# amolchanov86/gym_art

Measured on AMD Instinct MI355X. Metric: env-steps/sec (whole node) at N=2^20 Hummingbird; achieved HBM GB/s, higher is better.
Workload: dtype f64

## Files before the change

gym_art_amd/csrc/gaq.hip:

```cpp
#include "gaq_host.hpp"

#define GAQ_X(FEAT) extern template __global__ GAQ_STEP_SIG(FEAT)
GAQ_STEP_ALL(GAQ_X)
#undef GAQ_X
#define GAQ_X(FEAT) extern template __global__ GAQ_ROLL_SIG(FEAT)
GAQ_ROLL_ALL(GAQ_X)
#undef GAQ_X

namespace {

using namespace gaqk;

__global__ __launch_bounds__(kBlock) void episode_kernel(int64_t n, const float* __restrict__ reward,
                                                          const uint8_t* __restrict__ done, float* __restrict__ ep_ret,
                                                          uint32_t* __restrict__ ep_len, double* __restrict__ acc) {
  const int64_t i = (int64_t)blockIdx.x * kBlock + threadIdx.x;
  float ret = 0.0f; uint32_t len = 0; bool fin = false;
  if (i < n) {
    ret = ep_ret[i] + reward[i];
    len = ep_len[i] + 1u;
    fin = done[i] != 0;
    ep_ret[i] = fin ? 0.0f : ret;
    ep_len[i] = fin ? 0u : len;
  }
// ... 28 lines not shown
  for (int o = 32; o > 0; o >>= 1) acc += __shfl_down(acc, o);
  if ((threadIdx.x & 63) == 0) atomicAdd(reinterpret_cast<unsigned long long*>(out), (unsigned long long)acc);
}

__global__ __launch_bounds__(kBlock) void hbm_copy_kernel(const u32x4* __restrict__ src, u32x4* __restrict__ dst, size_t n16) {
  size_t i = (size_t)blockIdx.x * kBlock + threadIdx.x;
  const size_t stride = (size_t)gridDim.x * kBlock;
  for (; i < n16; i += stride) dst[i] = src[i];
}

__global__ void bump_kernel(uint64_t* ctr, uint64_t inc) { *ctr += inc; }
__global__ void fold_counter_kernel(uint64_t* ctr) {
  uint64_t sum = 0;
  for (int k = 0; k < kCtrSlots; ++k) { sum += ctr[k * kCtrStride]; ctr[k * kCtrStride] = 0; }
  ctr[0] = sum;
}

struct TileDirect {
  const DevPtrs& p; int64_t tile; uint32_t lane;
  __device__ __forceinline__ double ld64(const double* arr, int planes, int plane) const {
    auto r = __builtin_amdgcn_make_buffer_rsrc(const_cast<double*>(arr + tile * planes * kTile), 0, planes * kTile * 8, 0x00020000);
    return __builtin_bit_cast(double, __builtin_amdgcn_raw_buffer_load_b64(r, lane * 8u, plane * (kTile * 8), 0));
  }
  __device__ __forceinline__ void st64(double* arr, int planes, int plane, double v) const {
    auto r = __builtin_amdgcn_make_buffer_rsrc(arr + tile * planes * kTile, 0, planes * kTile * 8, 0x00020000);
    __builtin_amdgcn_raw_buffer_store_b64(__builtin_bit_cast(u32x2, v), r, lane * 8u, plane * (kTile * 8), 0);
  }
  __device__ __forceinline__ float ld32(const float* arr, int plane) const {
    auto r = __builtin_amdgcn_make_buffer_rsrc(const_cast<float*>(arr + tile * 4 * kTile), 0, kGrpBytes, 0x00020000);
    return __builtin_bit_cast(float, __builtin_amdgcn_raw_buffer_load_b32(r, lane * 4u, plane * (kTile * 4), 0));
// ... 27 lines not shown
      for (int k = 0; k < 18; ++k) v[k] = lo_decode(alias, p.obs_in, p.lo, i, k);
#pragma unroll
      for (int j = 0; j < 3; ++j) { s.pos[j] = v[j] + s.goal[j]; s.vel[j] = v[3 + j]; s.omega[j] = v[15 + j]; }
#pragma unroll
      for (int j = 0; j < 9; ++j) s.rot[j] = v[6 + j];
    } else {
#pragma unroll
      for (int j = 0; j < 3; ++j) { s.pos[j] = t.ld64(p.core, kCorePlanes, j); s.vel[j] = t.ld64(p.core, kCorePlanes, 3 + j);
                                    s.omega[j] = t.ld64(p.core, kCorePlanes, 15 + j); }
#pragma unroll
      for (int j = 0; j < 9; ++j) s.rot[j] = t.ld64(p.core, kCorePlanes, 6 + j);
    }
#pragma unroll
    for (int j = 0; j < 4; ++j) { s.rot_damp[j] = t.ld64(p.lag, kLagPlanes, j); s.cmds_damp[j] = t.ld32(p.cmds, j);
                                  s.ou[j] = t.ld32(p.ou, j); s.act_prev[j] = t.ld32(p.actp, j); }
    const uint32_t cw = p.ctr[i];
    s.tick = cw & 0xFFFFu; s.svd_ctr = cw >> 16;
    float acc[3] = {0.0f, 0.0f, 9.81f};
    float hist[4] = {s.act_prev[0], s.act_prev[1], s.act_prev[2], s.act_prev[3]};
    if (do_reset && (mask == nullptr || mask[i])) {
      gaq::reset_env<double, gaq::F_GENERIC>(s, cfg, cfg.env_offset + (uint64_t)i, cfg.step_index);
#pragma unroll
      for (int j = 0; j < 3; ++j) t.st32(p.goal, j, (float)s.goal[j]);
      if (!alias) {
#pragma unroll
        for (int j = 0; j < 3; ++j) { t.st64(p.core, kCorePlanes, j, s.pos[j]); t.st64(p.core, kCorePlanes, 3 + j, s.vel[j]);
                                      t.st64(p.core, kCorePlanes, 15 + j, s.omega[j]); }
#pragma unroll
        for (int j = 0; j < 9; ++j) t.st64(p.core, kCorePlanes, 6 + j, s.rot[j]);
      }
#pragma unroll
      for (int j = 0; j < 4; ++j) { t.st64(p.lag, kLagPlanes, j, s.rot_damp[j]); t.st32(p.cmds, j, s.cmds_damp[j]);
                                    t.st32(p.actp, j, s.act_prev[j]); }
      p.ctr[i] = (s.tick & 0xFFFFu) | (s.svd_ctr << 16);
      hist[0] = hist[1] = hist[2] = hist[3] = 0.0f;
    }
    float hi18[18];
#pragma unroll
    for (int k = 0; k < 18; ++k) hi18[k] = 0.0f;
    if (alias) {
      double v[18];
#pragma unroll
      for (int j = 0; j < 3; ++j) { v[j] = s.pos[j] - s.goal[j]; v[3 + j] = s.vel[j]; v[15 + j] = s.omega[j]; }
#pragma unroll
      for (int j = 0; j < 9; ++j) v[6 + j] = s.rot[j];
#pragma unroll
      for (int k = 0; k < 18; ++k) {
        if (alias == 2) { hi18[k] = (float)v[k]; }
        else { lo_encode(alias, p.lo, i, k, v[k]); hi18[k] = split_hi(v[k]); }
      }
// ... 364 lines not shown
    return fail(GAQ_ERR_STATE, "obs_state_alias: the observation tensor returned by the previous step / reset was modified before "
                               "this call -- it is the integrator state's fp32 head (include/gaq.h gaq_config.obs_state_alias); "
                               "copy it before editing, or create the handle with obs_state_alias = 2 (library-owned heads)");
  return GAQ_OK;
}

uint32_t launch_variant_of(const gaq_env* e) {
  const uint32_t v = (uint32_t)e->variant;
  if (e->d.rows_out && rows_twin_of(v) != 0xFFFFFFFFu) return rows_twin_of(v);
  if (e->d.step_ctr && ctr_twin_of(v) != 0xFFFFFFFFu) return ctr_twin_of(v);
  return v;
}

}

int launch_step(gaq_env* e, const float* actions, float* obs, float* reward, uint8_t* done, hipStream_t st) {
  e->info_valid = false;
  if ((reinterpret_cast<uintptr_t>(actions) & 15) != 0) return fail(GAQ_ERR_INVALID, "actions must be 16-byte aligned");
  if ((reinterpret_cast<uintptr_t>(obs) & 15) != 0) return fail(GAQ_ERR_INVALID, "obs must be 16-byte aligned");
  if (e->sc.noise == gaq::NOISE_INPUT) {
    if (!e->noise_next) return fail(GAQ_ERR_STATE, "GAQ_NOISE_INPUT: call gaq_set_noise_input_dev before each step");
    e->d.noise_in = e->noise_next;
    e->noise_next = nullptr;
  }
  if (e->sc.sense_input) {
    if (!e->sense_next) return fail(GAQ_ERR_STATE, "sense_input: call gaq_set_sense_input_dev before each step");
    e->d.sense_in = e->sense_next;
    e->sense_next = nullptr;
  }
  const int tiles_per_block = kBlock / kTile;
// ... 16 lines not shown
    const void* fn = step_kernel_ptr((uint32_t)e->variant);
    if (!fn || lds > 160 * 1024) return fail(GAQ_ERR_INVALID, "observation rows too large for the CU's LDS");
    HIP_TRY(hipFuncSetAttribute(fn, hipFuncAttributeMaxDynamicSharedMemorySize, (int)lds));
    e->lds_raised_for = e->variant;
  }
  const uint32_t launch_variant = launch_variant_of(e);
  if (e->d.rz_every > 0 && (launch_variant & gaq::F_RZ) != 0) {
    const bool hot_only = e->sc.compact_params != 0 && e->sc.zero_damp != 0 && (launch_variant & gaq::F_FP32) == 0;
    if (hot_only) e->cold_stale = true;
    else if (e->cold_stale) {
      if (int rc = launch_catch_up(e, st)) return rc;
    }
  }
  if (e->d.rz_every > 0 && e->rz_refill_now) { if (int rc = launch_refill(e, st)) return rc; }
  const bool self_counting = (launch_variant & gaq::F_CTR) != 0;
  if (e->d.step_ctr && !self_counting) {
    bool capturing = false;
    hipStreamCaptureStatus cs = hipStreamCaptureStatusNone;
    if (hipStreamIsCapturing(st, &cs) == hipSuccess) capturing = cs == hipStreamCaptureStatusActive; else (void)hipGetLastError();
    if (e->ctr_spread || capturing) {
      hipLaunchKernelGGL(fold_counter_kernel, dim3(1), dim3(1), 0, st, e->d.step_ctr);
      HIP_TRY(hipGetLastError());
      if (!capturing) e->ctr_spread = false;
    }
  }
  if (launch_variant != e->noted_step) { launch_record().note(0, launch_variant); e->noted_step = launch_variant; }
#define GAQ_LAUNCH(FEAT) \
  hipLaunchKernelGGL(step_kernel<(FEAT)>, grid, block, lds, st, e->d, e->sc, e->um, actions, obs, reward, done, lpw)
  switch (launch_variant) {
#define GAQ_X(FEAT) case (int)(FEAT): GAQ_LAUNCH(FEAT); break;
    GAQ_STEP_ALL(GAQ_X)
#undef GAQ_X
    default: return fail(GAQ_ERR_STATE, "internal: no kernel instantiation for this feature mask");
  }
// ... 116 lines not shown
float* mirror_aux(const gaq_env* e, char* base) { return reinterpret_cast<float*>(base + planes_bytes(e)); }

char* device_view(char* pinned) {
  void* dp = nullptr;
  if (hipHostGetDevicePointer(&dp, pinned, 0) == hipSuccess && dp) return static_cast<char*>(dp);
  (void)hipGetLastError();
  return nullptr;
}

int export_state(gaq_env* e, double* planes_dst, float* aux_dst, hipStream_t st) {
  if (!planes_dst) {
    if (!e->export_dev) HIP_TRY(hipMalloc((void**)&e->export_dev, planes_bytes(e)));
    planes_dst = e->export_dev;
  }
  if (e->alias) e->d.obs_in = e->last_obs;
  const dim3 grid((unsigned)((e->d.n + kBlock - 1) / kBlock)), block(kBlock);
  hipLaunchKernelGGL(export_kernel, grid, block, 0, st, e->d, alias_mode(e), planes_dst, aux_dst);
  HIP_TRY(hipGetLastError());
  return GAQ_OK;
}

int mirror_info(gaq_env* e) {
  if (!e->info_pin) {
    const bool mapped = e->stage_map != nullptr;
    HIP_TRY(hipHostMalloc((void**)&e->info_pin, planes_bytes(e) + aux_bytes(e), mapped ? hipHostMallocMapped : hipHostMallocDefault));
    if (mapped) e->info_map = device_view(e->info_pin);
  }
  if (e->info_map) return export_state(e, mirror_planes(e->info_map), mirror_aux(e, e->info_map), e->stream);
  if (int rc = export_state(e, nullptr, nullptr, e->stream)) return rc;
  HIP_TRY(hipMemcpyAsync(mirror_planes(e->info_pin), e->export_dev, planes_bytes(e), hipMemcpyDeviceToHost, e->stream));
// ... 81 lines not shown
    derive_model(cfg->model, dt, e->um);
    e->um.jinv = nullptr;
    if (cfg->control == GAQ_CTRL_MELLINGER && !inverse_jacobian(cfg->model, sc.jinv)) {
      delete e;
      return fail(GAQ_ERR_INVALID, "singular quadrotor jacobian");
    }
  } else {
    std::memset(&e->um, 0, sizeof(e->um));
  }
  { const ParamFlags f = start_flags(*cfg, e->um); e->any_lag = f.lag; e->any_drag = f.drag; }
  { const char* nf = getenv("GAQ_NO_FUSED"); if (nf && nf[0] == '1') e->fused_rollout = false; }
  e->ov = read_overrides();
  e->lomix = cfg->per_env_params != 0 || e->any_lag;
  { const char* ca = getenv("GAQ_CHECK_ALIAS"); e->check_alias = ca && ca[0] == '1'; }
  { const int sw = env_override("GAQ_SWEEP"); sc.sweep = sw < 0 ? kSweepDefault : sw; }
  {
    const char* ab = getenv("GAQ_ABLATE");
    sc.ablate = ab ? atoi(ab) : 0;
    if (sc.ablate != 0 && !kDiagBuild) {
      delete e;
      return fail(GAQ_ERR_INVALID, "GAQ_ABLATE is set but this libgaq is not a measurement build (make EXTRA=-DGAQ_DIAG_BUILD OUT=...): "
                                   "the ablations skip parts of the step and give wrong physics; unset the variable");
    }
    if (sc.ablate != 0) fprintf(stderr, "libgaq: GAQ_ABLATE=%d in a measurement build -- results are WRONG by construction, only timings mean anything\n", sc.ablate);
  }
  refresh_feature_flags(e);
  if (e->fp32 && !e->alias) {
    delete e;
    return fail(GAQ_ERR_INVALID, "fp32_state needs the specialised kernels (18-word world-frame obs, RawControl, default reward terms)");
  }
// ... 20 lines not shown
  if (e->alias) {
    if (!e->fp32) alloc0((void**)&d.lo, nt * (e->lomix ? (size_t)kMixRowsBytes : (size_t)kLoRowsBytes));
    alloc0((void**)&e->own_obs, nt * kRowsBytes);
  } else {
    alloc0((void**)&d.core, nt * kCoreBytes);
  }
  alloc0((void**)&d.lag, nt * kLagBytes);
  alloc0((void**)&d.ou, nt * kGrpBytes);
  alloc0((void**)&d.cmds, nt * kGrpBytes);
  alloc0((void**)&d.actp, nt * kGrpBytes);
  alloc0((void**)&d.goal, nt * kGrpBytes);
  alloc0((void**)&d.gyro, nt * kGrpBytes);
  alloc0((void**)&e->step_ctr_mem, sizeof(uint64_t) * kCtrSlots * kCtrStride);
  alloc0((void**)&e->alias_sum_dev, sizeof(uint64_t));
  alloc0((void**)&d.ctr, nt * kTile * sizeof(uint32_t));
  alloc0((void**)&d.done_count, sizeof(uint32_t) * 2);
  alloc0((void**)&d.nan_count, sizeof(uint32_t));
  if (cfg->compact_done) alloc0((void**)&d.done_list, nt * kTile * sizeof(uint32_t));
  if (cfg->aux_outputs) alloc0((void**)&d.aux, nt * kTile * gaq::AUX_WORDS * sizeof(float));
  if (cfg->per_env_params) {
    double* par = nullptr;
    double* jinv_dev = nullptr;
    alloc0((void**)&par, nt * kParBytes);
    if (cfg->control == GAQ_CTRL_MELLINGER) alloc0((void**)&jinv_dev, nt * kTile * 16 * sizeof(double));
    d.par = par;
    d.jinv = jinv_dev;
    alloc0((void**)&d.traj, 4 * nt * kTile * sizeof(uint32_t));
    d.rcount = d.traj ? d.traj + nt * kTile : nullptr;
    d.rz_flag = d.traj ? d.traj + 2 * nt * kTile : nullptr;
    e->host_par.assign(nt * kPar * kTile, 1.0);
// ... 40 lines not shown
    if (cfg->per_env_params)
      HIP_TRY(hipMemcpy(const_cast<double*>(d.par), e->host_par.data(), e->host_par.size() * sizeof(double), hipMemcpyHostToDevice));
    return GAQ_OK;
  };
  if (int rc = init_state()) { gaq_destroy(e); return rc; }
  *out = e;
  return GAQ_OK;
}

int gaq_destroy(gaq_env* e) {
  if (!e) return GAQ_OK;
  (void)hipSetDevice(e->cfg.device);
  if (e->stream) (void)hipStreamSynchronize(e->stream);
  (void)hipDeviceSynchronize();
  (void)hipFree(e->d.core); (void)hipFree(e->d.lo); (void)hipFree(e->own_obs); (void)hipFree(e->d.lag); (void)hipFree(e->d.ou); (void)hipFree(e->d.cmds);
  (void)hipFree(e->d.actp); (void)hipFree(e->d.goal); (void)hipFree(e->d.gyro); (void)hipFree(e->step_ctr_mem); if (e->info_pin) (void)hipHostFree(e->info_pin); (void)hipFree(e->alias_sum_dev); (void)hipFree(e->d.ctr);
  (void)hipFree(e->d.done_count); (void)hipFree(e->d.nan_count); (void)hipFree(e->d.done_list);
  (void)hipFree(e->d.ep_ret); (void)hipFree(e->d.ep_len); (void)hipFree(e->d.ep_acc); (void)hipFree(e->d.aux);
  (void)hipFree(const_cast<double*>(e->d.par)); (void)hipFree(const_cast<double*>(e->d.jinv));
  (void)hipFree(e->d.traj); (void)hipFree(e->d.rz_overrun);
  (void)hipFree(e->stage_dev); (void)hipFree(e->export_dev);
  if (e->stage_pin) (void)hipHostFree(e->stage_pin);
  if (e->ev0) (void)hipEventDestroy(e->ev0);
  if (e->ev1) (void)hipEventDestroy(e->ev1);
  if (e->stream) (void)hipStreamDestroy(e->stream);
  delete e;
  return GAQ_OK;
}

int gaq_is_diag_build(void) { return kDiagBuild ? 1 : 0; }

// ... 267 lines not shown
        lo_encode(mode, lo.data(), i, k, v);
      }
    HIP_TRY(hipMemcpy(e->own_obs, hi.data(), hi.size() * 4, hipMemcpyHostToDevice));
    if (!e->fp32) HIP_TRY(hipMemcpy(e->d.lo, lo.data(), lo.size(), hipMemcpyHostToDevice));
    e->last_obs = e->own_obs;
  } else {
    HIP_TRY(hipMemcpy(e->d.core, core.data(), core.size() * 8, hipMemcpyHostToDevice));
  }
  HIP_TRY(hipMemcpy(e->d.lag, lag.data(), lag.size() * 8, hipMemcpyHostToDevice));
  HIP_TRY(hipMemcpy(e->d.ou, ou.data(), ou.size() * 4, hipMemcpyHostToDevice));
  HIP_TRY(hipMemcpy(e->d.cmds, cmds.data(), cmds.size() * 4, hipMemcpyHostToDevice));
  HIP_TRY(hipMemcpy(e->d.actp, actp.data(), actp.size() * 4, hipMemcpyHostToDevice));
  HIP_TRY(hipMemcpy(e->d.goal, goal.data(), goal.size() * 4, hipMemcpyHostToDevice));
  HIP_TRY(hipMemcpy(e->d.gyro, gyro.data(), gyro.size() * 4, hipMemcpyHostToDevice));
  HIP_TRY(hipMemcpy(e->d.ctr, c.data(), c.size() * 4, hipMemcpyHostToDevice));
  e->rz_refill_now = true;
  return GAQ_OK;
}

int gaq_done_list(gaq_env* e, uint32_t* idx_out, int64_t capacity, int64_t* count_out) {
  if (!e || !count_out) return fail(GAQ_ERR_INVALID, "null argument");
  if (!e->d.done_list) return fail(GAQ_ERR_STATE, "handle was created with compact_done = 0");
  HIP_TRY(hipSetDevice(e->cfg.device));
  HIP_TRY(hipStreamSynchronize(e->stream));
  if (int rc_ = sync_handle(e)) return rc_;
  uint64_t step = e->sc.step_index;
  if (e->d.step_ctr) { if (int rc_ = read_step_counter(e, &step)) return rc_; }
  if (step == 0) { *count_out = 0; return GAQ_OK; }
  uint32_t cnt = 0;
  HIP_TRY(hipMemcpy(&cnt, e->d.done_count + ((step - 1) & 1), sizeof(uint32_t), hipMemcpyDeviceToHost));
// ... 167 lines not shown
```

gym_art_amd/csrc/gaq_host.hpp:

```cpp
#pragma once

#include <hip/hip_runtime.h>

#include <algorithm>
#include <cmath>
#include <cstdio>
#include <cstdlib>
#include <cstring>
#include <functional>
#include <mutex>
#include <new>
#include <set>
#include <string>
#include <vector>

#include "gaq_kernels.hpp"
#include "../../include/gaq.h"

using namespace gaqk;

namespace {
struct Randomizer {
  int32_t sampler, every;
  double ratio[gaq::TL_COUNT];
// ... 24 lines not shown
  int lds_raised_for = -1; bool reset_lds_raised = false;
  hipStream_t user_stream = nullptr;
  bool user_stream_used = false;
  const float* sense_next = nullptr;
  std::vector<double> host_par;
  bool dev_params = false;
  bool rz_on = false;
  bool cold_stale = false;
  int rz_since_refill = 0;
  bool rz_refill_now = false;
  Randomizer rz;
  std::vector<uint8_t> pflags;
  int64_t cnt_lag = 0, cnt_drag = 0, cnt_noncompact = 0, cnt_damp = 0;
  bool any_lag = false, any_drag = false;
  Overrides ov;
  bool ctr_spread = false;
  int num_cus = 256;
  int variant = 0;
  int lds_per_wave = 0;
  bool needs_generic = false;
  bool fused_rollout = true;
  bool alias = false;
  bool pack = false;
  bool shadow = false;
  bool check_alias = false;
  uint64_t* alias_sum_dev = nullptr;
  uint64_t alias_sum = 0; bool alias_sum_valid = false;
  bool lomix = false;
  bool fp32 = false;
  float* own_obs = nullptr;
// ... 15 lines not shown
      return fail(GAQ_ERR_DEVICE, std::string(#expr) + ": " + hipGetErrorString(e_));      \
  } while (0)

struct LaunchRecord {
  std::mutex mu;
  std::set<uint32_t> seen[3];
  void note(int kind, uint32_t f) { std::lock_guard<std::mutex> g(mu); seen[kind].insert(f); }
};
LaunchRecord& launch_record();

int fail(int code, const std::string& msg);
int env_override(const char* name);
int launch_step(gaq_env* e, const float* actions, float* obs, float* reward, uint8_t* done, hipStream_t st);
uint32_t fused_variant(const gaq_env* e);
int fused_rollout(gaq_env* e, int32_t T, float* obs, hipStream_t st, const std::function<int()>& launch);
int sync_handle(gaq_env* e);
int check_overrun(gaq_env* e);
void refresh_feature_flags(gaq_env* e);

void derive_model(const gaq_model& g, double dt, Model<double>& m);
bool inverse_jacobian(const gaq_model& g, double out[16]);
int check_model(const gaq_model& g);
int launch_refill(gaq_env* e, hipStream_t st);
int launch_jinv(gaq_env* e, hipStream_t st, const uint8_t* done);
int launch_catch_up(gaq_env* e, hipStream_t st);
int rebuild_params(gaq_env* e);

struct Scratch {
  void* p = nullptr;
  ~Scratch() { if (p) (void)hipFree(p); }
// ... 12 lines not shown
```

gym_art_amd/csrc/gaq_kernels.hpp:

```cpp
#pragma once

#include <hip/hip_runtime.h>

#include <cstddef>
#include <cstdint>

#include "../../include/gaq.h"
#include "quad_core.hpp"
#include "quad_params_dev.hpp"

namespace gaqk {

#ifndef GAQ_LD_AUX
#define GAQ_LD_AUX 0
#endif
#ifndef GAQ_ST_AUX
#define GAQ_ST_AUX 0
#endif
#ifndef GAQ_ACT_AUX
#define GAQ_ACT_AUX 0
#endif
#ifndef GAQ_ACTION_AUX
#define GAQ_ACTION_AUX GAQ_ACT_AUX
#endif
// ... 27 lines not shown
constexpr int kLoRowsLds = 3 * 1024;
constexpr int kMixRowWords = 11;
constexpr int kMixRowBytes = kMixRowWords * 4;
constexpr int kMixRowsBytes = kTile * kMixRowBytes;
template <uint32_t F> constexpr bool kLoMix = (F & (gaq::F_PER_ENV | gaq::F_LAG)) != 0;
constexpr int kPar = 45;
constexpr int kParBytes = kPar * kTile * 8;
constexpr int kHotPlanes = 19;
constexpr int kParNextSkew = 544;
enum ParPlane { PP_MASS = 0, PP_INV_MASS = 1, PP_INERTIA = 2, PP_INV_INERTIA = 5, PP_THRUST_MAX = 8, PP_TORQUE_MAX = 12,
                PP_PROP_X = 16, PP_PROP_Y = 20, PP_PROP_Z = 24, PP_TAU_UP = 28, PP_TAU_DOWN = 29, PP_LINEARITY = 30,
                PP_ARM = 31, PP_VEL_DAMP = 32, PP_DAMP_Q = 33, PP_C_DRAG = 34, PP_C_ROLL = 35, PP_OU_SIGMA = 36,
                PP_T2T = 37, PP_MX = 38, PP_MY = 39, PP_COMX = 40, PP_COMY = 41, PP_COMPACT_OK = 42,
                PP_T_UP = 43, PP_T_DOWN = 44 };

struct DevPtrs {
  double* core;
  void* lo;
  const float* obs_in;
  float* obs_copy;
  float* hi_final;
  double* lag;
  float* ou;
  float* cmds;
  float* actp;
  float* goal;
  float* gyro;
  uint32_t* ctr;
  const double* par;
  const double* jinv;
  const float* noise_in;
  const float* sense_in;
  float* aux;
  uint32_t* done_list;
  uint32_t* done_count;
  uint32_t* nan_count;
  float* term_obs;
  float* ep_ret;
  uint32_t* ep_len;
  double* ep_acc;
  uint64_t* step_ctr;
  uint32_t ctr_shift;
  uint32_t ctr_inc0;
// ... 9 lines not shown

using gaq::EnvState;
using gaq::Model;
using gaq::StepCfg;

template <uint32_t F> struct RealOf { using type = double; };
#define GAQ_REAL_FP32(FEAT) template <> struct RealOf<(FEAT)> { using type = float; };
GAQ_REAL_FP32(48u) GAQ_REAL_FP32(49u) GAQ_REAL_FP32(50u) GAQ_REAL_FP32(51u) GAQ_REAL_FP32(52u) GAQ_REAL_FP32(53u) GAQ_REAL_FP32(54u) GAQ_REAL_FP32(55u)
#undef GAQ_REAL_FP32
template <uint32_t F> using Real = typename RealOf<F>::type;

typedef unsigned int u32x2 __attribute__((ext_vector_type(2)));
typedef unsigned int u32x4 __attribute__((ext_vector_type(4)));
typedef __attribute__((address_space(3))) void lds_void;

struct TileImage { int lo, lag, ou, cmds, actp, goal, gyro, total; };

template <uint32_t F>
__host__ __device__ __forceinline__ TileImage tile_image(const StepCfg& cfg) {
  TileImage t;
  t.lo = kRowsLds;
  int o = (F & gaq::F_FP32) ? kRowsLds : (F & gaq::F_ALIAS) ? kRowsLds + kLoRowsLds : kCoreBytes;
  t.lag = o;  if (gaq::has_lag<F>(cfg)) o += kLagBytes;
  t.ou = o;   if (gaq::noise_mode<F>(cfg) != gaq::NOISE_OFF) o += kGrpBytes;
  t.cmds = o; if (gaq::has_lag<F>(cfg)) o += kGrpBytes;
  t.actp = o; if (gaq::has_act_prev<F>(cfg)) o += kGrpBytes;
  t.goal = o; if (gaq::has_env_goal<F>(cfg)) o += kGrpBytes;
  t.gyro = o; if (gaq::has_gyro_bias<F>(cfg)) o += kGrpBytes;
  t.total = o;
  return t;
// ... 506 lines not shown
template <uint32_t F> constexpr int kArgPrologue = 2;
#define GAQ_ARG_PROLOGUE(FEAT, FORM) template <> inline constexpr int kArgPrologue<(FEAT)> = (FORM);
GAQ_ARG_PROLOGUE(66578u, 1) GAQ_ARG_PROLOGUE(66577u, 1) GAQ_ARG_PROLOGUE(68627u, 1) GAQ_ARG_PROLOGUE(19477u, 1) GAQ_ARG_PROLOGUE(197653u, 1)
GAQ_ARG_PROLOGUE(197654u, 1) GAQ_ARG_PROLOGUE(197655u, 1) GAQ_ARG_PROLOGUE(199699u, 1)
#undef GAQ_ARG_PROLOGUE
template <uint32_t F, int FORM = 2, typename C, typename A>
__device__ __forceinline__ C kernarg_batch(uint32_t token, C carry, const DevPtrs& p, A actions, int lds_per_wave) {
  if constexpr (FORM == 1) {
    asm("s_waitcnt lgkmcnt(0)" : "+s"(carry) : "s"(token), "s"(p.ntiles), "s"(p.n), "s"(p.step_ctr));
    return carry;
  }
  if constexpr ((F & gaq::F_GENERIC) == 0) {
    if constexpr ((F & gaq::F_LAG) != 0) asm("" : "+s"(carry) : "s"(p.lag), "s"(p.cmds));
    if constexpr ((F & gaq::F_NOISE) != 0) asm("" : "+s"(carry) : "s"(p.ou));
  }
  if constexpr ((F & gaq::F_ALIAS) != 0) {
    asm("s_waitcnt lgkmcnt(0)" : "+s"(carry) : "s"(token), "s"(p.ntiles), "s"(p.n), "s"(p.step_ctr), "s"(p.ctr_shift), "s"(p.obs_in), "s"(p.lo),
        "s"(p.ctr), "s"(actions), "s"(lds_per_wave));
  } else {
    asm("s_waitcnt lgkmcnt(0)" : "+s"(carry) : "s"(token), "s"(p.ntiles), "s"(p.n), "s"(p.step_ctr), "s"(p.ctr_shift), "s"(p.core), "s"(p.ctr),
        "s"(actions), "s"(lds_per_wave));
  }
  return carry;
}

template <uint32_t F> constexpr int kStepMinWaves = 1;
#ifndef GAQ_NO_FLOORS
template <> inline constexpr int kStepMinWaves<214036u> = 3;
template <> inline constexpr int kStepMinWaves<82962u> = 3;
#endif
constexpr uint32_t kXcds = 8;
template <uint32_t F> constexpr bool kSweeps = true;
template <> inline constexpr bool kSweeps<17428u> = false;
template <> inline constexpr bool kSweeps<2569u> = false;
template <uint32_t F>
__global__ __launch_bounds__(kBlock) __attribute__((amdgpu_waves_per_eu(kStepMinWaves<F>))) void step_kernel(DevPtrs p, StepCfg cfg, Model<double> um,
// ... 15 lines not shown
      const uint32_t nblocks = (uint32_t)((p.ntiles + (kBlock / kTile - 1)) / (kBlock / kTile));
      const uint32_t xcd = block % kXcds, members = (nblocks - xcd + (kXcds - 1u)) / kXcds;
      const uint32_t mirrored = xcd + (members - 1u - block / kXcds) * kXcds;
      block = ((uint32_t)cfg.sweep & (uint32_t)cfg.step_index & 1u) != 0 ? mirrored : block;
    }
  }
  const int64_t tile = (int64_t)block * (kBlock / kTile) + wave;
  if constexpr ((F & gaq::F_CTR) != 0) {
    if (tile >= p.ntiles) {
      (void)step_counter_checkin(p, step_counter_read(p, lane), lane);
      return;
    }
  } else {
    if (tile >= p.ntiles) return;
  }
  char* buf = smem + wave * lds_per_wave;
  const int64_t i = tile * kTile + lane;
  const bool live = i < p.n;
  const int D = cfg.obs_dim;

  stage_in<F>(p, cfg, tile, buf, lane);
  if constexpr (kArgPrologue<F> == 2) __builtin_amdgcn_sched_barrier(0);
  using T = Real<F>;
  Model<T> m;
  if constexpr (!gaq::kModelMem<F>) load_model<F>(p, cfg, tile, lane, um, m);
  const Model<T>* mp = &m;
  if constexpr (gaq::kModelMem<F>) mp = (const Model<T>*)kernarg_model_ptr();
  float4 a4;
  uint32_t cw;
  {
    auto ra = __builtin_amdgcn_make_buffer_rsrc(const_cast<float*>(actions), 0, (int)(p.n * 16), 0x00020000);
    const u32x4 v = __builtin_amdgcn_raw_buffer_load_b128(ra, (uint32_t)i * 16u, 0, (F & gaq::F_NT) ? 2 : GAQ_ACTION_AUX);
    a4 = __builtin_bit_cast(float4, v);
    auto rc = __builtin_amdgcn_make_buffer_rsrc(p.ctr, 0, (int)(p.ntiles * kTile * 4), 0x00020000);
    cw = __builtin_amdgcn_raw_buffer_load_b32(rc, (uint32_t)i * 4u, 0, (F & gaq::F_NT) ? 2 : GAQ_ACT_AUX);
  }
  if constexpr ((F & gaq::F_CTR) != 0) cfg.step_index = step_counter_checkin(p, step_counter_read(p, lane), lane);
  float pre0[4] = {0.0f, 0.0f, 0.0f, 0.0f}, pre1[4] = {0.0f, 0.0f, 0.0f, 0.0f};
  if constexpr ((F & gaq::F_PREDRAW) != 0) {
    const gaq::Philox r0(cfg.seed, cfg.env_offset + (uint64_t)i, cfg.step_index, gaq::RNG_OU0);
    gaq::normals4(r0, pre0);
    if (cfg.sim_steps > 1) { const gaq::Philox r1(cfg.seed, cfg.env_offset + (uint64_t)i, cfg.step_index, gaq::RNG_OU0 + 1u); gaq::normals4(r1, pre1); }
  }
  if constexpr ((F & gaq::F_PREDRAW) != 0) {
    asm volatile("" :: "v"(pre0[0]), "v"(pre0[1]), "v"(pre0[2]), "v"(pre0[3]), "v"(pre1[0]), "v"(pre1[1]), "v"(pre1[2]), "v"(pre1[3]));
  }
  wait_dma();
  EnvState<T> s;
  read_image<F>(cfg, buf, lane, s);
  s.tick = cw & 0xFFFFu;
// ... 66 lines not shown
#pragma unroll
        for (int j = 0; j < 4; ++j) s.ou[j] = 0.0f;
      }
    }
  }
  if constexpr (kObsRowsInLds) {
    wave_lds_fence();
    if constexpr (A) flush_obs(p.obs_copy, p.n, D, tile, rows, lane);
    else flush_obs(obs, p.n, D, tile, rows, lane);
    if constexpr (kAuxRowsInLds) { if (p.aux) flush_obs(p.aux, p.n, gaq::AUX_WORDS, tile, rows + aux_off, lane); }
    wave_lds_fence();
  }
  write_image<F>(cfg, buf, lane, s);
  wave_lds_fence();
  stage_out<F>(p, cfg, tile, buf, lane, obs);
  {
    auto rc = __builtin_amdgcn_make_buffer_rsrc(p.ctr, 0, (int)(p.ntiles * kTile * 4), 0x00020000);
    __builtin_amdgcn_raw_buffer_store_b32((s.tick & 0xFFFFu) | (s.svd_ctr << 16), rc, (uint32_t)i * 4u, 0, kStAux<F>);
  }
  if (live) {
    if constexpr (GAQ_OUT_NT != 0) { __builtin_nontemporal_store(out.reward, &reward[i]); __builtin_nontemporal_store(out.done, &done[i]); }
    else { reward[i] = out.reward; done[i] = out.done; }
    if (!isfinite(out.reward)) atomicAdd(p.nan_count, 1u);
  }
  if constexpr (!gaq::kHeadsAreObs<F> && !kObsRowsInLds) {
    float* obs_rows_out = obs;
    if constexpr (A) obs_rows_out = p.obs_copy;
    wave_lds_fence();
    float* row = reinterpret_cast<float*>(rows) + lane * D;
    if (D == 18) {
#pragma unroll
// ... 169 lines not shown
  if (p.step_ctr) cfg.step_index = step_counter_peek(p, lane);
  const int64_t tile = (int64_t)blockIdx.x * (kBlock / kTile) + wave;
  if (tile >= p.ntiles) return;
  char* buf = smem + wave * lds_per_wave;
  const int64_t i = tile * kTile + lane;
  const bool live = i < p.n;
  const int64_t first = tile * kTile;
  const uint32_t nlive = (uint32_t)((p.n - first) < kTile ? (p.n - first) : kTile);
  const TileImage im = tile_image<F>(cfg);

  stage_in<F>(p, cfg, tile, buf, lane);
  __builtin_amdgcn_sched_barrier(0);
  using RT = Real<F>;
  Model<RT> m;
  load_model<F, true>(p, cfg, tile, lane, um, m);
  auto rc = __builtin_amdgcn_make_buffer_rsrc(p.ctr, 0, (int)(p.ntiles * kTile * 4), 0x00020000);
  const uint32_t cw = __builtin_amdgcn_raw_buffer_load_b32(rc, (uint32_t)i * 4u, 0, 0);
  auto load_action = [&](int t) {
    auto ra = __builtin_amdgcn_make_buffer_rsrc(const_cast<float*>(actions + ((int64_t)t * p.n + first) * 4), 0,
                                                (int)(nlive * 16u), 0x00020000);
    return __builtin_amdgcn_raw_buffer_load_b128(ra, lane * 16u, 0, 0);
  };
  u32x4 a_next = load_action(0);
  wait_dma();
  EnvState<RT> s;
  read_image<F>(cfg, buf, lane, s);
  s.tick = cw & 0xFFFFu;
  s.svd_ctr = cw >> 16;
  wave_lds_fence();
  StepCfg c = cfg;
  for (int t = 0; t < T; ++t) {
    const float4 a4 = __builtin_bit_cast(float4, a_next);
// ... 38 lines not shown
    wave_lds_fence();
    c.step_index += 1;
  }
  write_image<F>(cfg, buf, lane, s);
  wave_lds_fence();
  if (p.hi_final) copy_out_rows<5, kRowsBytes>(p.hi_final + first * 18, buf, lane, nlive * kRowBytes);
  if constexpr ((F & gaq::F_FP32) == 0) {
    if constexpr (kLoMix<F>) copy_out_rows<3, kMixRowsBytes>(reinterpret_cast<uint32_t*>(p.lo) + first * kMixRowWords, buf + im.lo, lane, kMixRowsBytes);
    else copy_out_rows<3, kLoRowsBytes>(reinterpret_cast<int16_t*>(p.lo) + first * 18, buf + im.lo, lane, kLoRowsBytes);
  }
  if (gaq::has_lag<F>(cfg)) {
    copy_out<2>(p.lag + tile * (kLagPlanes * kTile), buf + im.lag, lane);
    copy_out<1>(p.cmds + tile * (4 * kTile), buf + im.cmds, lane);
  }
  if (gaq::noise_mode<F>(cfg) != gaq::NOISE_OFF) copy_out<1>(p.ou + tile * (4 * kTile), buf + im.ou, lane);
  __builtin_amdgcn_raw_buffer_store_b32((s.tick & 0xFFFFu) | (s.svd_ctr << 16), rc, (uint32_t)i * 4u, 0, 0);
}

template <uint32_t F>
__device__ __forceinline__ void policy_rollout_body(const DevPtrs& p, StepCfg cfg, const Model<double>& um, int T, float* obs,
                                                    float* __restrict__ reward, uint8_t* __restrict__ done, char* buf, int64_t tile,
                                                    uint32_t lane, const PolicyDev* pol, float* pol_scratch, float* __restrict__ act_out) {
  const int64_t i = tile * kTile + lane;
  const bool live = i < p.n;
  const int64_t first = tile * kTile;
  const uint32_t nlive = (uint32_t)((p.n - first) < kTile ? (p.n - first) : kTile);
  const TileImage im = tile_image<F>(cfg);

  stage_in<F>(p, cfg, tile, buf, lane);
  using RT = Real<F>;
  Model<RT> m;
  load_model<F, true>(p, cfg, tile, lane, um, m);
  auto rc = __builtin_amdgcn_make_buffer_rsrc(p.ctr, 0, (int)(p.ntiles * kTile * 4), 0x00020000);
  const uint32_t cw = __builtin_amdgcn_raw_buffer_load_b32(rc, (uint32_t)i * 4u, 0, 0);
  wait_dma();
  EnvState<RT> s;
  read_image<F>(cfg, buf, lane, s);
  s.tick = cw & 0xFFFFu;
  s.svd_ctr = cw >> 16;
  wave_lds_fence();
  StepCfg c = cfg;
  for (int t = 0; t < T; ++t) {
    float act[4];
    policy_eval(*pol, reinterpret_cast<const float*>(buf + lane * kRowBytes), pol_scratch, lane, c.seed, c.env_offset + (uint64_t)i,
                c.step_index, act);
    if (act_out && live) {
      const u32x4 v = __builtin_bit_cast(u32x4, make_float4(act[0], act[1], act[2], act[3]));
      auto ro = __builtin_amdgcn_make_buffer_rsrc(act_out + ((int64_t)t * p.n + first) * 4, 0, (int)(nlive * 16u), 0x00020000);
      __builtin_amdgcn_raw_buffer_store_b128(v, ro, lane * 16u, 0, 0);
// ... 37 lines not shown
    wave_lds_fence();
    c.step_index += 1;
  }
  write_image<F>(cfg, buf, lane, s);
  wave_lds_fence();
  if (p.hi_final) copy_out_rows<5, kRowsBytes>(p.hi_final + first * 18, buf, lane, nlive * kRowBytes);
  if constexpr ((F & gaq::F_FP32) == 0) {
    if constexpr (kLoMix<F>) copy_out_rows<3, kMixRowsBytes>(reinterpret_cast<uint32_t*>(p.lo) + first * kMixRowWords, buf + im.lo, lane, kMixRowsBytes);
    else copy_out_rows<3, kLoRowsBytes>(reinterpret_cast<int16_t*>(p.lo) + first * 18, buf + im.lo, lane, kLoRowsBytes);
  }
  if (gaq::has_lag<F>(cfg)) {
    copy_out<2>(p.lag + tile * (kLagPlanes * kTile), buf + im.lag, lane);
    copy_out<1>(p.cmds + tile * (4 * kTile), buf + im.cmds, lane);
  }
  if (gaq::noise_mode<F>(cfg) != gaq::NOISE_OFF) copy_out<1>(p.ou + tile * (4 * kTile), buf + im.ou, lane);
  __builtin_amdgcn_raw_buffer_store_b32((s.tick & 0xFFFFu) | (s.svd_ctr << 16), rc, (uint32_t)i * 4u, 0, 0);
}

constexpr int kPolBlock = kTile;
template <uint32_t F>
__global__ __launch_bounds__(kPolBlock) void policy_rollout_kernel(DevPtrs p, StepCfg cfg, Model<double> um, int T, PolicyDev pol,
                                                                   float* __restrict__ act_out, float* obs, float* __restrict__ reward,
                                                                   uint8_t* __restrict__ done, int lds_per_wave) {
  static_assert((F & gaq::F_ALIAS) != 0 && (F & gaq::F_GENERIC) == 0, "fused rollout: alias layout only");
  extern __shared__ __attribute__((aligned(16))) char smem[];
  const uint32_t lane = threadIdx.x & 63u;
  const int64_t tile = kernarg_batch<F>(kernarg_warm(), (int64_t)blockIdx.x, p, act_out, lds_per_wave);
  if (p.step_ctr) cfg.step_index = step_counter_peek(p, lane);
  if (tile >= p.ntiles) return;
  float* scratch = reinterpret_cast<float*>(smem + ((lds_per_wave + 15) & ~15));
  policy_rollout_body<F>(p, cfg, um, T, obs, reward, done, smem, tile, lane, &pol, scratch, act_out);
// ... 41 lines not shown
```

gym_art_amd/csrc/gaq_params.hip:

```cpp
#include "gaq_host.hpp"

namespace {

dim3 grid_for(int64_t count) { return dim3((unsigned)((count + kBlock - 1) / kBlock)); }

__global__ __launch_bounds__(kBlock) void clear_dynamics_kernel(DevPtrs p, const int64_t* __restrict__ idx, int64_t first, int64_t count) {
  const int64_t k = (int64_t)blockIdx.x * kBlock + threadIdx.x;
  if (k >= count) return;
  const int64_t i = idx ? idx[k] : first + k;
  p.ctr[i] &= 0xFFFFu;
  float* ou = p.ou + (i / kTile) * (4 * kTile) + (i % kTile);
#pragma unroll
  for (int j = 0; j < 4; ++j) ou[j * kTile] = 0.0f;
}

__device__ __forceinline__ uint32_t* pfull_of(const DevPtrs& p) { return p.traj + 3 * p.ntiles * kTile; }

struct PlaneDest { double* base; int lane, stride; };
__device__ __forceinline__ PlaneDest env_planes(const DevPtrs& p, int64_t i) {
  return {const_cast<double*>(p.par) + (i / kTile) * (int64_t)(kPar * kTile), (int)(i % kTile), kTile};
}
__device__ __forceinline__ PlaneDest plane_row(double* row) { return {row, 0, 1}; }

__device__ __forceinline__ void write_model_planes(const PlaneDest& to, double dt, const gaq::DerivedModel& dm) {
// ... 342 lines not shown
    std::sort(tiles.begin(), tiles.end());
    tiles.erase(std::unique(tiles.begin(), tiles.end()), tiles.end());
    for (size_t a = 0; a < tiles.size();) {
      size_t b = a + 1;
      while (b < tiles.size() && tiles[b] == tiles[b - 1] + 1) ++b;
      HIP_TRY(hipMemcpy(const_cast<double*>(e->d.par) + (size_t)tiles[a] * kPar * kTile, hp + (size_t)tiles[a] * kPar * kTile,
                        (b - a) * (size_t)kParBytes, hipMemcpyHostToDevice));
      a = b;
    }
  }
  Scratch di;
  if (idx) {
    if (di.alloc(sizeof(int64_t) * (size_t)count)) return GAQ_ERR_DEVICE;
    HIP_TRY(hipMemcpy(di.p, idx, sizeof(int64_t) * (size_t)count, hipMemcpyHostToDevice));
  }
  hipLaunchKernelGGL(clear_dynamics_kernel, grid_for(count), dim3(kBlock), 0, e->stream, e->d, (const int64_t*)di.p, first, count);
  HIP_TRY(hipGetLastError());
  HIP_TRY(hipStreamSynchronize(e->stream));
  flags_from_counts(e);
  return GAQ_OK;
}

int need_device_params(gaq_env* e) {
  if (!e) return fail(GAQ_ERR_INVALID, "null handle");
  if (!e->cfg.per_env_params) return fail(GAQ_ERR_STATE, "handle was created with per_env_params = 0");
  return GAQ_OK;
}
int check_tree(const gaq_quad_params& t, bool by_density = false) {
  const double* v = reinterpret_cast<const double*>(&t);
  for (int k = 0; k < GAQ_TREE_DOUBLES; ++k) if (!std::isfinite(v[k])) return fail(GAQ_ERR_INVALID, "parameter tree: non-finite leaf");
// ... 55 lines not shown
  }
  e->d.rz_every = e->d.par_next ? rz->every : 0;
  e->rz_refill_now = true;
  const uint8_t nf = rz->sampler == 2 ? (uint8_t)PF_LAG : tree_flags(rz->base, e->sc.dt);
  for (int64_t i = 0; i < e->d.n; ++i) set_env_flags(e, i, nf);
  flags_from_counts(e);
  return GAQ_OK;
}

int gaq_randomize_dev(gaq_env* e, const uint8_t* mask_dev, void* stream) {
  if (int rc = need_device_params(e)) return rc;
  e->info_valid = false;
  if (!e->rz_on) return fail(GAQ_ERR_STATE, "no randomizer installed (gaq_set_randomizer)");
  HIP_TRY(hipSetDevice(e->cfg.device));
  e->user_stream = (hipStream_t)stream; e->user_stream_used = true;
  hipLaunchKernelGGL(params_redraw_kernel, grid_for(e->d.n), dim3(kBlock), 0, (hipStream_t)stream, e->d, e->sc, e->rz, mask_dev);
  HIP_TRY(hipGetLastError());
  if (int rc = launch_jinv(e, (hipStream_t)stream, nullptr)) return rc;
  if (e->d.rz_every > 0) return launch_refill(e, (hipStream_t)stream);
  return GAQ_OK;
}

int gaq_set_param_trees(gaq_env* e, const gaq_quad_params* trees, int32_t links_by_density, int64_t first, int64_t count) {
  if (int rc = need_device_params(e)) return rc;
  e->info_valid = false;
  if (!trees) return fail(GAQ_ERR_INVALID, "null argument");
  if (int rc = check_range(e, first, count)) return rc;
  if (count == 0) return GAQ_OK;
  if (!e->dev_params && (e->cnt_lag | e->cnt_drag | e->cnt_noncompact | e->cnt_damp) != 0)
    return fail(GAQ_ERR_STATE, "this handle already holds host-supplied parameters (gaq_set_params): do not mix the two paths");
  for (int64_t k = 0; k < count; ++k) if (int rc = check_tree(trees[k], links_by_density != 0)) return rc;
  HIP_TRY(hipSetDevice(e->cfg.device));
  if (int rc_ = sync_handle(e)) return rc_;
  Scratch dt_;
  if (dt_.alloc(sizeof(gaq_quad_params) * (size_t)count)) return GAQ_ERR_DEVICE;
  HIP_TRY(hipMemcpy(dt_.p, trees, sizeof(gaq_quad_params) * (size_t)count, hipMemcpyHostToDevice));
  hipLaunchKernelGGL(derive_trees_kernel, grid_for(count), dim3(kBlock), 0, e->stream, e->d, e->sc, (const double*)dt_.p, (int)links_by_density, first, count);
  HIP_TRY(hipGetLastError());
  e->dev_params = true;
  if (int rc = launch_jinv(e, e->stream, nullptr)) return rc;
  HIP_TRY(hipStreamSynchronize(e->stream));
  for (int64_t k = 0; k < count; ++k) set_env_flags(e, first + k, tree_flags(trees[k], e->sc.dt));
  flags_from_counts(e);
  return GAQ_OK;
}

int gaq_get_params(gaq_env* e, gaq_model* out, int64_t first, int64_t count) {
  if (!e || !out) return fail(GAQ_ERR_INVALID, "null argument");
  if (!e->cfg.per_env_params) return fail(GAQ_ERR_STATE, "handle was created with per_env_params = 0");
  if (int rc = check_range(e, first, count)) return rc;
  if (count == 0) return GAQ_OK;
// ... 46 lines not shown
```

Before: 22.62 billion.

## Elide per-env counter traffic with per-tile uniform counter headers

```diff
diff --git a/gym_art_amd/csrc/gaq.hip b/gym_art_amd/csrc/gaq.hip
--- a/gym_art_amd/csrc/gaq.hip
+++ b/gym_art_amd/csrc/gaq.hip
@@ -66,6 +66,16 @@
   uint64_t sum = 0;
   for (int k = 0; k < kCtrSlots; ++k) { sum += ctr[k * kCtrStride]; ctr[k * kCtrStride] = 0; }
   ctr[0] = sum;
+}
+
+__global__ __launch_bounds__(kBlock) void ctr_materialise_kernel(DevPtrs p) {
+  const int64_t i = (int64_t)blockIdx.x * kBlock + threadIdx.x;
+  const int64_t tile = i / kTile;
+  if (tile >= p.ntiles) return;
+  const CtrHdr h = p.ctr_hdr[tile];
+  if (h.uniform == 0) return;
+  p.ctr[i] = h.cw;
+  if (i % kTile == 0) const_cast<CtrHdr*>(p.ctr_hdr)[tile] = CtrHdr{0u, 0u};
 }
 
 struct TileDirect {
@@ -123,7 +133,8 @@
 #pragma unroll
     for (int j = 0; j < 4; ++j) { s.rot_damp[j] = t.ld64(p.lag, kLagPlanes, j); s.cmds_damp[j] = t.ld32(p.cmds, j);
                                   s.ou[j] = t.ld32(p.ou, j); s.act_prev[j] = t.ld32(p.actp, j); }
-    const uint32_t cw = p.ctr[i];
+    const CtrHdr ch = p.ctr_hdr[tile];
+    const uint32_t cw = ch.uniform ? ch.cw : p.ctr[i];
     s.tick = cw & 0xFFFFu; s.svd_ctr = cw >> 16;
     float acc[3] = {0.0f, 0.0f, 9.81f};
     float hist[4] = {s.act_prev[0], s.act_prev[1], s.act_prev[2], s.act_prev[3]};
@@ -141,8 +152,11 @@
 #pragma unroll
       for (int j = 0; j < 4; ++j) { t.st64(p.lag, kLagPlanes, j, s.rot_damp[j]); t.st32(p.cmds, j, s.cmds_damp[j]);
                                     t.st32(p.actp, j, s.act_prev[j]); }
-      p.ctr[i] = (s.tick & 0xFFFFu) | (s.svd_ctr << 16);
       hist[0] = hist[1] = hist[2] = hist[3] = 0.0f;
+    }
+    if (do_reset) {
+      if (ch.uniform || mask == nullptr || mask[i]) p.ctr[i] = (s.tick & 0xFFFFu) | (s.svd_ctr << 16);
+      if (ch.uniform && lane == 0) const_cast<CtrHdr*>(p.ctr_hdr)[tile] = CtrHdr{0u, 0u};
     }
     float hi18[18];
 #pragma unroll
@@ -537,6 +551,34 @@
 
 }
 
+namespace {
+bool step_reads_ctr_hdr(uint32_t f) {
+  switch (f) {
+#define GAQ_X(FEAT) case (FEAT):
+    GAQ_CTR_PLANE_ONLY(GAQ_X)
+#undef GAQ_X
+      return false;
+    default: return true;
+  }
+}
+bool stream_capturing(hipStream_t st) {
+  hipStreamCaptureStatus cs = hipStreamCaptureStatusNone;
+  if (hipStreamIsCapturing(st, &cs) == hipSuccess) return cs == hipStreamCaptureStatusActive;
+  (void)hipGetLastError();
+  return false;
+}
+}
+
+int materialise_ctr(gaq_env* e, hipStream_t st) {
+  if (!e->ctr_elide) return GAQ_OK;
+  const bool capturing = stream_capturing(st);
+  if (!(e->ctr_stale || capturing)) return GAQ_OK;
+  hipLaunchKernelGGL(ctr_materialise_kernel, dim3((unsigned)((e->d.ntiles * kTile + kBlock - 1) / kBlock)), dim3(kBlock), 0, st, e->d);
+  HIP_TRY(hipGetLastError());
+  if (!capturing && !e->ctr_captured) e->ctr_stale = false;
+  return GAQ_OK;
+}
+
 int launch_step(gaq_env* e, const float* actions, float* obs, float* reward, uint8_t* done, hipStream_t st) {
   e->info_valid = false;
   if ((reinterpret_cast<uintptr_t>(actions) & 15) != 0) return fail(GAQ_ERR_INVALID, "actions must be 16-byte aligned");
@@ -583,10 +625,14 @@
   }
   if (e->d.rz_every > 0 && e->rz_refill_now) { if (int rc = launch_refill(e, st)) return rc; }
   const bool self_counting = (launch_variant & gaq::F_CTR) != 0;
+  if (e->ctr_elide && step_reads_ctr_hdr(launch_variant)) {
+    e->ctr_stale = true;
+    if (!e->ctr_captured) e->ctr_captured = stream_capturing(st);
+  } else if (e->ctr_stale) {
+    if (int rc = materialise_ctr(e, st)) return rc;
+  }
   if (e->d.step_ctr && !self_counting) {
-    bool capturing = false;
-    hipStreamCaptureStatus cs = hipStreamCaptureStatusNone;
-    if (hipStreamIsCapturing(st, &cs) == hipSuccess) capturing = cs == hipStreamCaptureStatusActive; else (void)hipGetLastError();
+    const bool capturing = stream_capturing(st);
     if (e->ctr_spread || capturing) {
       hipLaunchKernelGGL(fold_counter_kernel, dim3(1), dim3(1), 0, st, e->d.step_ctr);
       HIP_TRY(hipGetLastError());
@@ -733,6 +779,7 @@
     planes_dst = e->export_dev;
   }
   if (e->alias) e->d.obs_in = e->last_obs;
+  if (int rc = materialise_ctr(e, st)) return rc;
   const dim3 grid((unsigned)((e->d.n + kBlock - 1) / kBlock)), block(kBlock);
   hipLaunchKernelGGL(export_kernel, grid, block, 0, st, e->d, alias_mode(e), planes_dst, aux_dst);
   HIP_TRY(hipGetLastError());
@@ -844,6 +891,8 @@
   e->lomix = cfg->per_env_params != 0 || e->any_lag;
   { const char* ca = getenv("GAQ_CHECK_ALIAS"); e->check_alias = ca && ca[0] == '1'; }
   { const int sw = env_override("GAQ_SWEEP"); sc.sweep = sw < 0 ? kSweepDefault : sw; }
+  e->ctr_elide = env_override("GAQ_CTR_ELIDE") != 0;
+  if (e->ctr_elide) sc.sweep |= 2;
   {
     const char* ab = getenv("GAQ_ABLATE");
     sc.ablate = ab ? atoi(ab) : 0;
@@ -894,6 +943,7 @@
   alloc0((void**)&e->step_ctr_mem, sizeof(uint64_t) * kCtrSlots * kCtrStride);
   alloc0((void**)&e->alias_sum_dev, sizeof(uint64_t));
   alloc0((void**)&d.ctr, nt * kTile * sizeof(uint32_t));
+  alloc0((void**)&d.ctr_hdr, nt * sizeof(CtrHdr));
   alloc0((void**)&d.done_count, sizeof(uint32_t) * 2);
   alloc0((void**)&d.nan_count, sizeof(uint32_t));
   if (cfg->compact_done) alloc0((void**)&d.done_list, nt * kTile * sizeof(uint32_t));
@@ -964,7 +1014,7 @@
   if (e->stream) (void)hipStreamSynchronize(e->stream);
   (void)hipDeviceSynchronize();
   (void)hipFree(e->d.core); (void)hipFree(e->d.lo); (void)hipFree(e->own_obs); (void)hipFree(e->d.lag); (void)hipFree(e->d.ou); (void)hipFree(e->d.cmds);
-  (void)hipFree(e->d.actp); (void)hipFree(e->d.goal); (void)hipFree(e->d.gyro); (void)hipFree(e->step_ctr_mem); if (e->info_pin) (void)hipHostFree(e->info_pin); (void)hipFree(e->alias_sum_dev); (void)hipFree(e->d.ctr);
+  (void)hipFree(e->d.actp); (void)hipFree(e->d.goal); (void)hipFree(e->d.gyro); (void)hipFree(e->step_ctr_mem); if (e->info_pin) (void)hipHostFree(e->info_pin); (void)hipFree(e->alias_sum_dev); (void)hipFree(e->d.ctr); (void)hipFree(const_cast<CtrHdr*>(e->d.ctr_hdr));
   (void)hipFree(e->d.done_count); (void)hipFree(e->d.nan_count); (void)hipFree(e->d.done_list);
   (void)hipFree(e->d.ep_ret); (void)hipFree(e->d.ep_len); (void)hipFree(e->d.ep_acc); (void)hipFree(e->d.aux);
   (void)hipFree(const_cast<double*>(e->d.par)); (void)hipFree(const_cast<double*>(e->d.jinv));
@@ -1262,6 +1312,8 @@
   HIP_TRY(hipMemcpy(e->d.goal, goal.data(), goal.size() * 4, hipMemcpyHostToDevice));
   HIP_TRY(hipMemcpy(e->d.gyro, gyro.data(), gyro.size() * 4, hipMemcpyHostToDevice));
   HIP_TRY(hipMemcpy(e->d.ctr, c.data(), c.size() * 4, hipMemcpyHostToDevice));
+  HIP_TRY(hipMemset(const_cast<CtrHdr*>(e->d.ctr_hdr), 0, nt * sizeof(CtrHdr)));
+  if (!e->ctr_captured) e->ctr_stale = false;
   e->rz_refill_now = true;
   return GAQ_OK;
 }
diff --git a/gym_art_amd/csrc/gaq_host.hpp b/gym_art_amd/csrc/gaq_host.hpp
--- a/gym_art_amd/csrc/gaq_host.hpp
+++ b/gym_art_amd/csrc/gaq_host.hpp
@@ -62,6 +62,9 @@
   int64_t cnt_lag = 0, cnt_drag = 0, cnt_noncompact = 0, cnt_damp = 0;
   bool any_lag = false, any_drag = false;
   Overrides ov;
+  bool ctr_elide = true;
+  bool ctr_stale = false;
+  bool ctr_captured = false;
   bool ctr_spread = false;
   int num_cus = 256;
   int variant = 0;
@@ -107,6 +110,7 @@
 int launch_step(gaq_env* e, const float* actions, float* obs, float* reward, uint8_t* done, hipStream_t st);
 uint32_t fused_variant(const gaq_env* e);
 int fused_rollout(gaq_env* e, int32_t T, float* obs, hipStream_t st, const std::function<int()>& launch);
+int materialise_ctr(gaq_env* e, hipStream_t st);
 int sync_handle(gaq_env* e);
 int check_overrun(gaq_env* e);
 void refresh_feature_flags(gaq_env* e);
diff --git a/gym_art_amd/csrc/gaq_kernels.hpp b/gym_art_amd/csrc/gaq_kernels.hpp
--- a/gym_art_amd/csrc/gaq_kernels.hpp
+++ b/gym_art_amd/csrc/gaq_kernels.hpp
@@ -65,6 +65,8 @@
                 PP_T2T = 37, PP_MX = 38, PP_MY = 39, PP_COMX = 40, PP_COMY = 41, PP_COMPACT_OK = 42,
                 PP_T_UP = 43, PP_T_DOWN = 44 };
 
+struct CtrHdr { uint32_t cw, uniform; };
+
 struct DevPtrs {
   double* core;
   void* lo;
@@ -78,6 +80,7 @@
   float* goal;
   float* gyro;
   uint32_t* ctr;
+  const CtrHdr* ctr_hdr;
   const double* par;
   const double* jinv;
   const float* noise_in;
@@ -117,6 +120,33 @@
 typedef unsigned int u32x4 __attribute__((ext_vector_type(4)));
 typedef __attribute__((address_space(3))) void lds_void;
 
+__device__ __forceinline__ CtrHdr ctr_hdr_load(const DevPtrs& p, int64_t tile) {
+  const CtrHdr h = p.ctr_hdr[tile];
+  return {(uint32_t)__builtin_amdgcn_readfirstlane((int)h.cw), (uint32_t)__builtin_amdgcn_readfirstlane((int)h.uniform)};
+}
+constexpr bool ctr_elide_on(const StepCfg& cfg) { return (cfg.sweep & 2) != 0; }
+template <int AUX>
+__device__ __forceinline__ uint32_t ctr_load(const DevPtrs& p, const CtrHdr h, int64_t i) {
+  const bool uni = h.uniform != 0;
+  auto rc = __builtin_amdgcn_make_buffer_rsrc(p.ctr, 0, uni ? 0 : (int)(p.ntiles * kTile * 4), 0x00020000);
+  return __builtin_amdgcn_raw_buffer_load_b32(rc, (uint32_t)i * 4u, 0, AUX) | (uni ? h.cw : 0u);
+}
+template <int AUX>
+__device__ __forceinline__ void ctr_store(const DevPtrs& p, const CtrHdr h, int64_t tile, uint32_t lane, uint32_t w, bool may_elide) {
+  const uint32_t w0 = (uint32_t)__builtin_amdgcn_readfirstlane((int)w);
+  const bool uni = may_elide && __ballot(w != w0) == 0ull;
+  auto rc = __builtin_amdgcn_make_buffer_rsrc(p.ctr, 0, uni ? 0 : (int)(p.ntiles * kTile * 4), 0x00020000);
+  __builtin_amdgcn_raw_buffer_store_b32(w, rc, (uint32_t)(tile * kTile + lane) * 4u, 0, AUX);
+  auto rh = __builtin_amdgcn_make_buffer_rsrc(const_cast<CtrHdr*>(p.ctr_hdr + tile), 0, (uni || h.uniform != 0) ? (int)sizeof(CtrHdr) : 0, 0x00020000);
+  const u32x2 hv = {uni ? w0 : 0u, uni ? 1u : 0u};
+  __builtin_amdgcn_raw_buffer_store_b64(hv, rh, lane * (uint32_t)sizeof(CtrHdr), 0, AUX);
+}
+#define GAQ_CTR_PLANE_ONLY(X) X(17424u) X(66578u) X(459794u) X(2569u) X(33812u)
+template <uint32_t F> constexpr bool kCtrHdr = true;
+#define GAQ_X(FEAT) template <> inline constexpr bool kCtrHdr<(FEAT)> = false;
+GAQ_CTR_PLANE_ONLY(GAQ_X)
+#undef GAQ_X
+
 struct TileImage { int lo, lag, ou, cmds, actp, goal, gyro, total; };
 
 template <uint32_t F>
@@ -653,12 +683,20 @@
     if constexpr ((F & gaq::F_LAG) != 0) asm("" : "+s"(carry) : "s"(p.lag), "s"(p.cmds));
     if constexpr ((F & gaq::F_NOISE) != 0) asm("" : "+s"(carry) : "s"(p.ou));
   }
-  if constexpr ((F & gaq::F_ALIAS) != 0) {
+  if constexpr (!kCtrHdr<F>) {
+    if constexpr ((F & gaq::F_ALIAS) != 0) {
+      asm("s_waitcnt lgkmcnt(0)" : "+s"(carry) : "s"(token), "s"(p.ntiles), "s"(p.n), "s"(p.step_ctr), "s"(p.ctr_shift), "s"(p.obs_in), "s"(p.lo),
+          "s"(p.ctr), "s"(actions), "s"(lds_per_wave));
+    } else {
+      asm("s_waitcnt lgkmcnt(0)" : "+s"(carry) : "s"(token), "s"(p.ntiles), "s"(p.n), "s"(p.step_ctr), "s"(p.ctr_shift), "s"(p.core), "s"(p.ctr),
+          "s"(actions), "s"(lds_per_wave));
+    }
+  } else if constexpr ((F & gaq::F_ALIAS) != 0) {
     asm("s_waitcnt lgkmcnt(0)" : "+s"(carry) : "s"(token), "s"(p.ntiles), "s"(p.n), "s"(p.step_ctr), "s"(p.ctr_shift), "s"(p.obs_in), "s"(p.lo),
-        "s"(p.ctr), "s"(actions), "s"(lds_per_wave));
+        "s"(p.ctr), "s"(p.ctr_hdr), "s"(actions), "s"(lds_per_wave));
   } else {
     asm("s_waitcnt lgkmcnt(0)" : "+s"(carry) : "s"(token), "s"(p.ntiles), "s"(p.n), "s"(p.step_ctr), "s"(p.ctr_shift), "s"(p.core), "s"(p.ctr),
-        "s"(actions), "s"(lds_per_wave));
+        "s"(p.ctr_hdr), "s"(actions), "s"(lds_per_wave));
   }
   return carry;
 }
@@ -704,6 +742,8 @@
   } else {
     if (tile >= p.ntiles) return;
   }
+  CtrHdr hdr = {0u, 0u};
+  if constexpr (kCtrHdr<F>) hdr = ctr_hdr_load(p, tile);
   char* buf = smem + wave * lds_per_wave;
   const int64_t i = tile * kTile + lane;
   const bool live = i < p.n;
@@ -722,8 +762,12 @@
     auto ra = __builtin_amdgcn_make_buffer_rsrc(const_cast<float*>(actions), 0, (int)(p.n * 16), 0x00020000);
     const u32x4 v = __builtin_amdgcn_raw_buffer_load_b128(ra, (uint32_t)i * 16u, 0, (F & gaq::F_NT) ? 2 : GAQ_ACTION_AUX);
     a4 = __builtin_bit_cast(float4, v);
-    auto rc = __builtin_amdgcn_make_buffer_rsrc(p.ctr, 0, (int)(p.ntiles * kTile * 4), 0x00020000);
-    cw = __builtin_amdgcn_raw_buffer_load_b32(rc, (uint32_t)i * 4u, 0, (F & gaq::F_NT) ? 2 : GAQ_ACT_AUX);
+    if constexpr (kCtrHdr<F>) {
+      cw = ctr_load<(F & gaq::F_NT) ? 2 : GAQ_ACT_AUX>(p, hdr, i);
+    } else {
+      auto rc = __builtin_amdgcn_make_buffer_rsrc(p.ctr, 0, (int)(p.ntiles * kTile * 4), 0x00020000);
+      cw = __builtin_amdgcn_raw_buffer_load_b32(rc, (uint32_t)i * 4u, 0, (F & gaq::F_NT) ? 2 : GAQ_ACT_AUX);
+    }
   }
   if constexpr ((F & gaq::F_CTR) != 0) cfg.step_index = step_counter_checkin(p, step_counter_read(p, lane), lane);
   float pre0[4] = {0.0f, 0.0f, 0.0f, 0.0f}, pre1[4] = {0.0f, 0.0f, 0.0f, 0.0f};
@@ -820,7 +864,9 @@
   write_image<F>(cfg, buf, lane, s);
   wave_lds_fence();
   stage_out<F>(p, cfg, tile, buf, lane, obs);
-  {
+  if constexpr (kCtrHdr<F>) {
+    ctr_store<kStAux<F>>(p, hdr, tile, lane, (s.tick & 0xFFFFu) | (s.svd_ctr << 16), ctr_elide_on(cfg) && (tile + 1) * kTile <= p.n);
+  } else {
     auto rc = __builtin_amdgcn_make_buffer_rsrc(p.ctr, 0, (int)(p.ntiles * kTile * 4), 0x00020000);
     __builtin_amdgcn_raw_buffer_store_b32((s.tick & 0xFFFFu) | (s.svd_ctr << 16), rc, (uint32_t)i * 4u, 0, kStAux<F>);
   }
@@ -1020,8 +1066,8 @@
   using RT = Real<F>;
   Model<RT> m;
   load_model<F, true>(p, cfg, tile, lane, um, m);
-  auto rc = __builtin_amdgcn_make_buffer_rsrc(p.ctr, 0, (int)(p.ntiles * kTile * 4), 0x00020000);
-  const uint32_t cw = __builtin_amdgcn_raw_buffer_load_b32(rc, (uint32_t)i * 4u, 0, 0);
+  const CtrHdr hdr = ctr_hdr_load(p, tile);
+  const uint32_t cw = ctr_load<0>(p, hdr, i);
   auto load_action = [&](int t) {
     auto ra = __builtin_amdgcn_make_buffer_rsrc(const_cast<float*>(actions + ((int64_t)t * p.n + first) * 4), 0,
                                                 (int)(nlive * 16u), 0x00020000);
@@ -1090,7 +1136,7 @@
     copy_out<1>(p.cmds + tile * (4 * kTile), buf + im.cmds, lane);
   }
   if (gaq::noise_mode<F>(cfg) != gaq::NOISE_OFF) copy_out<1>(p.ou + tile * (4 * kTile), buf + im.ou, lane);
-  __builtin_amdgcn_raw_buffer_store_b32((s.tick & 0xFFFFu) | (s.svd_ctr << 16), rc, (uint32_t)i * 4u, 0, 0);
+  ctr_store<0>(p, hdr, tile, lane, (s.tick & 0xFFFFu) | (s.svd_ctr << 16), false);
 }
 
 template <uint32_t F>
@@ -1107,8 +1153,8 @@
   using RT = Real<F>;
   Model<RT> m;
   load_model<F, true>(p, cfg, tile, lane, um, m);
-  auto rc = __builtin_amdgcn_make_buffer_rsrc(p.ctr, 0, (int)(p.ntiles * kTile * 4), 0x00020000);
-  const uint32_t cw = __builtin_amdgcn_raw_buffer_load_b32(rc, (uint32_t)i * 4u, 0, 0);
+  const CtrHdr hdr = ctr_hdr_load(p, tile);
+  const uint32_t cw = ctr_load<0>(p, hdr, i);
   wait_dma();
   EnvState<RT> s;
   read_image<F>(cfg, buf, lane, s);
@@ -1176,7 +1222,7 @@
     copy_out<1>(p.cmds + tile * (4 * kTile), buf + im.cmds, lane);
   }
   if (gaq::noise_mode<F>(cfg) != gaq::NOISE_OFF) copy_out<1>(p.ou + tile * (4 * kTile), buf + im.ou, lane);
-  __builtin_amdgcn_raw_buffer_store_b32((s.tick & 0xFFFFu) | (s.svd_ctr << 16), rc, (uint32_t)i * 4u, 0, 0);
+  ctr_store<0>(p, hdr, tile, lane, (s.tick & 0xFFFFu) | (s.svd_ctr << 16), false);
 }
 
 constexpr int kPolBlock = kTile;
diff --git a/gym_art_amd/csrc/gaq_params.hip b/gym_art_amd/csrc/gaq_params.hip
--- a/gym_art_amd/csrc/gaq_params.hip
+++ b/gym_art_amd/csrc/gaq_params.hip
@@ -380,6 +380,7 @@
     if (di.alloc(sizeof(int64_t) * (size_t)count)) return GAQ_ERR_DEVICE;
     HIP_TRY(hipMemcpy(di.p, idx, sizeof(int64_t) * (size_t)count, hipMemcpyHostToDevice));
   }
+  if (int rc = materialise_ctr(e, e->stream)) return rc;
   hipLaunchKernelGGL(clear_dynamics_kernel, grid_for(count), dim3(kBlock), 0, e->stream, e->d, (const int64_t*)di.p, first, count);
   HIP_TRY(hipGetLastError());
   HIP_TRY(hipStreamSynchronize(e->stream));
@@ -465,6 +466,7 @@
   if (!e->rz_on) return fail(GAQ_ERR_STATE, "no randomizer installed (gaq_set_randomizer)");
   HIP_TRY(hipSetDevice(e->cfg.device));
   e->user_stream = (hipStream_t)stream; e->user_stream_used = true;
+  if (int rc = materialise_ctr(e, (hipStream_t)stream)) return rc;
   hipLaunchKernelGGL(params_redraw_kernel, grid_for(e->d.n), dim3(kBlock), 0, (hipStream_t)stream, e->d, e->sc, e->rz, mask_dev);
   HIP_TRY(hipGetLastError());
   if (int rc = launch_jinv(e, (hipStream_t)stream, nullptr)) return rc;
@@ -486,6 +488,7 @@
   Scratch dt_;
   if (dt_.alloc(sizeof(gaq_quad_params) * (size_t)count)) return GAQ_ERR_DEVICE;
   HIP_TRY(hipMemcpy(dt_.p, trees, sizeof(gaq_quad_params) * (size_t)count, hipMemcpyHostToDevice));
+  if (int rc = materialise_ctr(e, e->stream)) return rc;
   hipLaunchKernelGGL(derive_trees_kernel, grid_for(count), dim3(kBlock), 0, e->stream, e->d, e->sc, (const double*)dt_.p, (int)links_by_density, first, count);
   HIP_TRY(hipGetLastError());
   e->dev_params = true;
```

Result: no change. 22.81 billion, median of 4 (+0.8%).
